# labhamlet/wavjepa

Hardware: AMD Instinct MI355X
Metric: jepa_pretrain_clips_per_sec (higher is better)
Workload: dtype bf16; 1 GPU; WavJEPA-base JEPA pre-training step, 2.01 s @16 kHz white-noise clips (32159 samples -> 200 tokens), 256 clips per GPU (32 sources x 8 crops), AudioSet masker, random-init weights; workload_name=2s-bf16, global_batch=256, seq_len=200, parallelism=dp1, persistent_gemm_workgroups_per_xcd=32

## Files before the change

include/wavjepa_hip.h:

```cpp
#ifndef WAVJEPA_HIP_H
#define WAVJEPA_HIP_H
#include <stdint.h>

#ifdef __cplusplus
extern "C" {
#endif

#define WJ_ABI_VERSION 17
int wj_abi_version(void);
int wj_device_count(void);
int wj_struct_size(const char* name);

enum {
    WJ_EPI_BF16 = 0,
    WJ_EPI_BIAS_GELU2 = 1,
    WJ_EPI_MUL_GELU_GRAD = 2,
    WJ_EPI_ADD_F32 = 3,
    WJ_EPI_ATOMIC_F32 = 4,
    WJ_EPI_CONV_GELU = 5,
    WJ_EPI_BIAS_GELU = 6,
    WJ_EPI_BF16_ADD_POS = 8,
    WJ_EPI_MUL_GELU_GRAD_Z = 7
};
typedef struct {
// ... 246 lines not shown
} wj_gelu_bwd_args;
int wj_gelu_bwd_bf16(const wj_gelu_bwd_args*, void* stream);

typedef struct {
    int64_t ticks;
} wj_spin_args;
int wj_spin(const wj_spin_args*, void* stream);


typedef struct {
    void* buf;
    const int32_t* rows;
    int32_t n_rows, row_bytes;
} wj_zero_rows_args;
int wj_zero_rows(const wj_zero_rows_args*, void* stream);

typedef struct {
    const void* src;
    void* dst;
    int32_t C_out, C_in, k, stride, rho, U, mode;
} wj_conv_w_args;
int wj_conv_weight_layout(const wj_conv_w_args*, void* stream);

typedef struct {
    const void* x;
    const float* pos;
    float* y_f32;
    void* y_bf16;
    int32_t M, T, D;
} wj_add_pos_args;
int wj_add_pos(const wj_add_pos_args*, void* stream);

typedef struct {
    const void* x;
    const int32_t* idx;
    void* out;
    int32_t n_rows, D, elem_bytes;
// ... 237 lines not shown
```

wavjepa_amd/csrc/conv0.hip:

```cpp
#include <string.h>
#include "common.h"
#include "../../include/wavjepa_hip.h"

namespace {

constexpr int TC = 256;
constexpr int NTH = 256;

struct Geo {
    int N, C_in, L, C, k, stride, L_out, P;
    long clip_stride;
};

template <int TAPS>
__device__ __forceinline__ void load_weights(float (&w)[4][TAPS], const bf16_t* __restrict__ wsrc, int c4) {
#pragma unroll
    for (int j = 0; j < 4; ++j)
#pragma unroll
        for (int tp = 0; tp < TAPS; ++tp) w[j][tp] = bf2f(wsrc[(long)(c4 + j) * TAPS + tp]);
}

__device__ __forceinline__ int stage_audio(float* xs, const bf16_t* __restrict__ audio, const Geo& g, int n, int t0, int span_max) {
    const int span = min(span_max, g.L - t0 * g.stride);
    for (int ci = 0; ci < g.C_in; ++ci)
// ... 44 lines not shown
    }
}

constexpr int STATS_SLOTS = 768;
inline int stats_tcs(int N, int L_out, int C_in) {
    static int forced = -1;
    if (forced < 0) forced = wj_lab_env_int("WJ_CONV0_STATS_TCS", 0);
    if (forced >= 32) return forced / 32 * 32;
    int chunks = (STATS_SLOTS + N / 2) / (N > 0 ? N : 1);
    const int most = (L_out + 255) / 256;
    chunks = chunks < 1 ? 1 : (chunks > most ? most : chunks);
    const int tcs = ((L_out + chunks - 1) / chunks + 31) / 32 * 32;
    const int cap = 2176 / (C_in > 0 ? C_in : 1) / 32 * 32;
    return tcs > cap ? (cap < 32 ? 32 : cap) : tcs;
}
template <int TAPS>
__global__ __launch_bounds__(256) void conv0_gram_kernel(const bf16_t* __restrict__ audio, double* __restrict__ part, Geo g, int span, int TCS) {
    extern __shared__ __attribute__((aligned(16))) bf16_t xa[];
    constexpr int G = TAPS + TAPS * TAPS;
    __shared__ double red[4][G];
    const int n = blockIdx.y, t0 = blockIdx.x * TCS;
    for (int ci = 0; ci < g.C_in; ++ci)
        for (int i = threadIdx.x; i < span; i += 256) {
            const long src = (long)t0 * g.stride + i;
            xa[ci * span + i] = src < g.L ? audio[(long)n * g.clip_stride + (long)ci * g.L + src] : f2bf(0.f);
        }
    __syncthreads();
    const int lane = threadIdx.x & 63, wave = threadIdx.x >> 6;
    const int tcount = min(TCS, g.L_out - t0);
    for (int p = lane; p < G; p += 64) {
        const bool one = p < TAPS;
        const int qa = one ? p : (p - TAPS) / TAPS, qb = one ? 0 : (p - TAPS) - qa * TAPS;
        const int ca = qa / g.k, cb = qb / g.k;
        const int offa = ca * span + (qa - ca * g.k), offb = cb * span + (qb - cb * g.k);
        double acc = 0.0;
        for (int t = wave; t < tcount; t += 4) {
            const float a = bf2f(xa[offa + t * g.stride]);
            const float b = one ? 1.0f : bf2f(xa[offb + t * g.stride]);
            acc += (double)(a * b);
        }
        red[wave][p] = acc;
    }
    __syncthreads();
    double* o = part + ((long)n * gridDim.x + blockIdx.x) * G;
    for (int p = threadIdx.x; p < G; p += 256) o[p] = (red[0][p] + red[1][p]) + (red[2][p] + red[3][p]);
}

__global__ __launch_bounds__(256) void conv0_fold_f64_kernel(const double* __restrict__ part, int chunks, int rec, double* __restrict__ out) {
    const int n = blockIdx.y;
    const double* src = part + (long)n * chunks * rec;
    for (int i = blockIdx.x * 256 + threadIdx.x; i < rec; i += gridDim.x * 256) {
        double s = 0.0;
        for (int ch = 0; ch < chunks; ++ch) s += src[(long)ch * rec + i];
        out[(long)n * rec + i] = s;
    }
}
// ... 568 lines not shown
```

wavjepa_amd/csrc/misc.hip:

```cpp
#include <string.h>
#include "common.h"
#include "../../include/wavjepa_hip.h"
#ifdef WJ_LAB
#include "../../include/wavjepa_hip_lab.h"
#endif

namespace {

inline int grid_for(long n_items, int per_block, int cap = 8192) {
    long g = (n_items + per_block - 1) / per_block;
    if (g < 1) g = 1;
    return (int)(g > cap ? cap : g);
}

__global__ __launch_bounds__(256) void gelu_bwd_kernel(const bf16_t* __restrict__ dpost, const bf16_t* __restrict__ pre,
                                                       bf16_t* __restrict__ dpre, long n8) {
    for (long i = blockIdx.x * 256L + threadIdx.x; i < n8; i += (long)gridDim.x * 256) {
        const bf16x8 d = *reinterpret_cast<const bf16x8*>(dpost + i * 8);
        const bf16x8 p = *reinterpret_cast<const bf16x8*>(pre + i * 8);
        bf16x8 o;
#pragma unroll
        for (int e = 0; e < 8; ++e) o[e] = f2bf(bf2f(d[e]) * gelu_grad_f(bf2f(p[e])));
        *reinterpret_cast<bf16x8*>(dpre + i * 8) = o;
    }
// ... 13 lines not shown
        for (int e = 0; e < 8; ++e) { o[e] = f2bf(bf2f(d[e]) * gelu_grad_f(bf2f(p[e]))); z[e] = f2bf(0.f); }
        *reinterpret_cast<bf16x8*>(dpre + off) = o;
        if (clear_dpost) *reinterpret_cast<bf16x8*>(dpost + off) = z;
    }
}

__global__ __launch_bounds__(256) void zero_rows_kernel(char* __restrict__ buf, const int32_t* __restrict__ rows, int n_rows,
                                                        int row16) {
    const long n = (long)n_rows * row16;
    for (long i = blockIdx.x * 256L + threadIdx.x; i < n; i += (long)gridDim.x * 256) {
        const int r = (int)(i / row16), c = (int)(i - (long)r * row16);
        *reinterpret_cast<uint4*>(buf + ((long)rows[r] * row16 + c) * 16) = make_uint4(0, 0, 0, 0);
    }
}

__global__ __launch_bounds__(256) void conv_w_kernel(wj_conv_w_args a) {
    const int Co = a.C_out, Ci = a.C_in, k = a.k;
    if (a.mode == 0) {
        const long n = (long)Co * Ci * k;
        for (long i = blockIdx.x * 256L + threadIdx.x; i < n; i += (long)gridDim.x * 256) {
            const int c = (int)(i % Ci);
            const int kk = (int)((i / Ci) % k);
            const int o = (int)(i / ((long)Ci * k));
            ((bf16_t*)a.dst)[i] = f2bf(((const float*)a.src)[((long)o * Ci + c) * k + kk]);
        }
    } else if (a.mode == 1) {
        const long n = (long)a.U * Co * Ci;
        for (long i = blockIdx.x * 256L + threadIdx.x; i < n; i += (long)gridDim.x * 256) {
            const int c = (int)(i % Ci);
            const int o = (int)((i / Ci) % Co);
            const int v = (int)(i / ((long)Ci * Co));
            const int kk = a.rho + a.stride * (a.U - 1 - v);
            ((bf16_t*)a.dst)[i] = f2bf(((const float*)a.src)[((long)o * Ci + c) * k + kk]);
        }
    } else {
        const long n = (long)Co * Ci * k;
        for (long i = blockIdx.x * 256L + threadIdx.x; i < n; i += (long)gridDim.x * 256) {
            const int kk = (int)(i % k);
            const int c = (int)((i / k) % Ci);
            const int o = (int)(i / ((long)Ci * k));
            ((float*)a.dst)[i] += ((const float*)a.src)[(long)o * Ci * k + (long)kk * Ci + c];
        }
    }
}

__global__ __launch_bounds__(256) void add_pos_kernel(wj_add_pos_args a) {
    const int D4 = a.D / 4;
    const long n = (long)a.M * D4;
    for (long i = blockIdx.x * 256L + threadIdx.x; i < n; i += (long)gridDim.x * 256) {
        const int m = (int)(i / D4), c = (int)(i - (long)m * D4) * 4;
        const bf16x4 x = *reinterpret_cast<const bf16x4*>((const bf16_t*)a.x + (long)m * a.D + c);
        const f32x4 p = *reinterpret_cast<const f32x4*>(a.pos + (long)(m % a.T) * a.D + c);
        f32x4 y;
        bf16x4 yb;
#pragma unroll
        for (int e = 0; e < 4; ++e) { y[e] = bf2f(x[e]) + p[e]; yb[e] = f2bf(y[e]); }
        if (a.y_f32) *reinterpret_cast<f32x4*>(a.y_f32 + (long)m * a.D + c) = y;
        if (a.y_bf16) *reinterpret_cast<bf16x4*>((bf16_t*)a.y_bf16 + (long)m * a.D + c) = yb;
// ... 452 lines not shown

extern "C" int wj_abi_version(void) { return WJ_ABI_VERSION; }
extern "C" int wj_device_count(void) {
    int n = 0;
    if (hipGetDeviceCount(&n) != hipSuccess) return 0;
    return n;
}

extern "C" int wj_struct_size(const char* name) {
    if (!name) return -1;
#define WJ_SZ(T) if (!strcmp(name, #T)) return (int)sizeof(T);
    WJ_SZ(wj_gemm_args) WJ_SZ(wj_ln_fwd_args) WJ_SZ(wj_ln_bwd_args) WJ_SZ(wj_ln_pre_fwd_args) WJ_SZ(wj_ln_pre_bwd_args) WJ_SZ(wj_colsum_args) WJ_SZ(wj_attn_fwd_args)
    WJ_SZ(wj_attn_bwd_args) WJ_SZ(wj_conv0_fwd_args) WJ_SZ(wj_conv0_bwd_args) WJ_SZ(wj_gelu_bwd_args) WJ_SZ(wj_conv_w_args)
    WJ_SZ(wj_add_pos_args) WJ_SZ(wj_gather_args) WJ_SZ(wj_scatter_fill_args) WJ_SZ(wj_scatter_fill_bwd_args)
    WJ_SZ(wj_unmask_rows_args) WJ_SZ(wj_instnorm_args) WJ_SZ(wj_mse_args) WJ_SZ(wj_ema_args) WJ_SZ(wj_sumsq_args)
    WJ_SZ(wj_adamw_args) WJ_SZ(wj_cast_args) WJ_SZ(wj_crop_args) WJ_SZ(wj_zero_rows_args) WJ_SZ(wj_instnorm_mean_args) WJ_SZ(wj_spin_args)
    WJ_SZ(wj_gemm_fp8_args) WJ_SZ(wj_quantize_fp8_args) WJ_SZ(wj_wgrad_group_args) WJ_SZ(wj_rir_conv_args) WJ_SZ(wj_snr_mix_args) WJ_SZ(wj_resample_args) WJ_SZ(wj_mse_groups_args) WJ_SZ(wj_transpose_args) WJ_SZ(wj_colsum_group_args) WJ_SZ(wj_rccl_init_args) WJ_SZ(wj_rccl_launch_args) WJ_SZ(wj_rccl_wait_args) WJ_SZ(wj_audio_prepare_args) WJ_SZ(wj_noise_prepare_args)
#ifdef WJ_LAB
    WJ_SZ(wj_collective_footprint_args)
#endif
#undef WJ_SZ
    return -1;
}

int64_t wj_gemm_ws_bytes(const wj_gemm_args* a);
int64_t wj_wgrad_group_ws_bytes(const wj_wgrad_group_args* a);
int64_t wj_colsum_bf16_ws_bytes(const wj_colsum_args* a);
int64_t wj_conv0_fwd_ws_bytes(const wj_conv0_fwd_args* a);
int64_t wj_conv0_bwd_ws_bytes(const wj_conv0_bwd_args* a);
int64_t wj_rir_conv_ws_bytes(const wj_rir_conv_args* a);
int64_t wj_snr_mix_ws_bytes(const wj_snr_mix_args* a);
// ... 19 lines not shown
    if (!strcmp(fn, "wj_conv0_gn_gelu_fwd")) return wj_conv0_fwd_ws_bytes((const wj_conv0_fwd_args*)args);
    if (!strcmp(fn, "wj_conv0_gn_gelu_bwd")) return wj_conv0_bwd_ws_bytes((const wj_conv0_bwd_args*)args);
    if (!strcmp(fn, "wj_masked_mse")) {
        const wj_mse_args* a = (const wj_mse_args*)args;
        return (2 + (int64_t)a->B * a->G * a->T) * 4;
    }
    if (!strcmp(fn, "wj_grad_sumsq")) return 1024 * 4;
    if (!strcmp(fn, "wj_rir_convolve")) return wj_rir_conv_ws_bytes((const wj_rir_conv_args*)args);
    if (!strcmp(fn, "wj_snr_mix")) return wj_snr_mix_ws_bytes((const wj_snr_mix_args*)args);
    if (!strcmp(fn, "wj_mse_groups")) return wj_mse_groups_ws_bytes((const wj_mse_groups_args*)args);
    if (!strcmp(fn, "wj_audio_prepare")) return wj_audio_prepare_ws_bytes((const wj_audio_prepare_args*)args);
    if (!strcmp(fn, "wj_noise_prepare")) return wj_noise_prepare_ws_bytes((const wj_noise_prepare_args*)args);
    static const char* const none[] = {"wj_layernorm_fwd", "wj_layernorm_pre_fwd", "wj_colsum_f32", "wj_attn_fwd", "wj_gelu_bwd_bf16",
        "wj_conv_weight_layout", "wj_add_pos", "wj_mask_gather_rows", "wj_mask_scatter_fill_pos",
        "wj_unmask_rows_f32", "wj_instnorm_accumulate", "wj_instnorm_mean", "wj_ema_update", "wj_adamw_step", "wj_cast_f32_to_bf16",
        "wj_crop_normalize_bf16", "wj_zero_rows", "wj_spin", "wj_gemm_mxfp8", "wj_quantize_mxfp8", "wj_resample_fir", "wj_transpose_bf16", "wj_colsum_f32_group", "wj_rccl_bucket_allreduce_launch", "wj_rccl_bucket_allreduce_wait", "wj_collective_footprint"};
    for (const char* n : none)
        if (!strcmp(fn, n)) return 0;
    return -1;
}

extern "C" int wj_gelu_bwd_bf16(const wj_gelu_bwd_args* a, void* stream) {
    WJ_CLEAR_STALE_ERROR();
    if (a && a->rows) {
        if (!a->dpost || !a->pre || !a->dpre || a->n_rows < 0 || a->row_elems <= 0 || (a->row_elems & 7)) return WJ_ERR_ARG;
        if (a->n_rows == 0) return WJ_OK;
        hipLaunchKernelGGL(gelu_bwd_rows_kernel, dim3(grid_for((long)a->n_rows * (a->row_elems / 8), 256)), dim3(256), 0, STREAM,
                           (bf16_t*)a->dpost, (const bf16_t*)a->pre, (bf16_t*)a->dpre, a->rows, a->n_rows, a->row_elems / 8,
                           a->clear_dpost);
        WJ_CHECK_LAUNCH();
        return WJ_OK;
// ... 60 lines not shown
    WJ_CHECK_LAUNCH();
    return WJ_OK;
}
#endif

extern "C" int wj_zero_rows(const wj_zero_rows_args* a, void* stream) {
    WJ_CLEAR_STALE_ERROR();
    if (!a || !a->buf || !a->rows || a->n_rows < 0 || a->row_bytes <= 0 || (a->row_bytes & 15)) return WJ_ERR_ARG;
    if (a->n_rows == 0) return WJ_OK;
    hipLaunchKernelGGL(zero_rows_kernel, dim3(grid_for((long)a->n_rows * (a->row_bytes / 16), 256)), dim3(256), 0, STREAM,
                       (char*)a->buf, a->rows, a->n_rows, a->row_bytes / 16);
    WJ_CHECK_LAUNCH();
    return WJ_OK;
}

extern "C" int wj_conv_weight_layout(const wj_conv_w_args* a, void* stream) {
    WJ_CLEAR_STALE_ERROR();
    if (!a || !a->src || !a->dst || a->C_out <= 0 || a->C_in <= 0 || a->k <= 0 || a->mode < 0 || a->mode > 2) return WJ_ERR_ARG;
    if (a->mode == 1 && (a->U <= 0 || a->rho < 0 || a->rho + a->stride * (a->U - 1) >= a->k)) return WJ_ERR_ARG;
    const long n = a->mode == 1 ? (long)a->U * a->C_out * a->C_in : (long)a->C_out * a->C_in * a->k;
    hipLaunchKernelGGL(conv_w_kernel, dim3(grid_for(n, 256, 2048)), dim3(256), 0, STREAM, *a);
    WJ_CHECK_LAUNCH();
    return WJ_OK;
}

extern "C" int wj_add_pos(const wj_add_pos_args* a, void* stream) {
    WJ_CLEAR_STALE_ERROR();
    if (!a || !a->x || !a->pos || a->M <= 0 || a->T <= 0 || a->D <= 0 || (a->D & 3)) return WJ_ERR_ARG;
    hipLaunchKernelGGL(add_pos_kernel, dim3(grid_for((long)a->M * a->D / 4, 256)), dim3(256), 0, STREAM, *a);
    WJ_CHECK_LAUNCH();
    return WJ_OK;
}

extern "C" int wj_mask_gather_rows(const wj_gather_args* a, void* stream) {
    WJ_CLEAR_STALE_ERROR();
    if (!a || !a->x || !a->idx || !a->out || a->n_rows < 0 || a->D <= 0) return WJ_ERR_ARG;
// ... 139 lines not shown
```

wavjepa_amd/engine.py:

```python
from __future__ import annotations

from dataclasses import dataclass
from typing import Dict, List, Optional, Sequence, Tuple

import numpy as np
import torch

from . import ops
from .params import FlatParams


def _empty(*shape, dtype, device):
    import os
    if os.environ.get("WJ_ARENA_FILL", "") == "nan":
        if not dtype.is_floating_point:
            return torch.full(shape, 0x7f, dtype=dtype, device=device)
        return torch.full(shape, float("nan"), dtype=dtype, device=device)
    return torch.empty(*shape, dtype=dtype, device=device)


@dataclass
class EngineConfig:
    conv_spec: Sequence[Tuple[int, int, int]]
    in_channels: int
# ... 250 lines not shown
        self.T = self.S * self.Tc
        self.stacks = list(cfg.conv_prefixes)
        assert len(self.stacks) in (1, self.S)
        self.C = cfg.conv_spec[-1][0]
        assert all(c == self.C for c, _, _ in cfg.conv_spec), "all conv layers must have the same width"
        assert cfg.d_enc % cfg.h_enc == 0 and cfg.d_dec % cfg.h_dec == 0
        self.N = 0
        self.G = 0
        import os as _os
        self.use_side = _os.environ.get("WJ_SIDE_STREAM", "1") != "0"
        self._opt_ev = None
        self.ragged = _os.environ.get("WJ_RAGGED", "1") != "0"
        self.ragged_step = False
        self.sparse_conv = _os.environ.get("WJ_SPARSE_CONV", "1") != "0" and all(k >= st for _, k, st in cfg.conv_spec[1:])
        self._conv_grads_dirty = False
        self.deterministic = _os.environ.get("WJ_DETERMINISTIC", "0") == "1"
        self._det_slab: Dict[str, torch.Tensor] = {}
        self.fuse_conv_gelu_bwd = _os.environ.get("WJ_FUSE_CONV_GELU_BWD", "1") != "0"
        self.trim_tail = _os.environ.get("WJ_TRIM_TAIL", "1") != "0"
        self.tail = None
        self.fp8 = _os.environ.get("WJ_FP8", "0") == "1"
        self._check_fp8()
        self._w8: Dict[int, Tuple[torch.Tensor, torch.Tensor, int, int]] = {}
        self._a8: Dict[str, Tuple[torch.Tensor, torch.Tensor]] = {}
        self.side = self._pick_side_stream() if self.use_side else torch.cuda.Stream(device=self.dev)
        self.has_mapper = "post_extraction_mapper.weight" in flat.by_name
        self.wt_dgrad = _os.environ.get("WJ_WT_DGRAD", "1") != "0"
        self.pair_split = _os.environ.get("WJ_PAIR_SPLIT", "0") == "1"
        self.pair_ws = None
        self._conv_w_fresh = False
# ... 149 lines not shown
                mine.copy_(src.reshape(mine.shape))
        if force_cast or not f.bf16_fresh:
            ops.cast_f32_to_bf16(f.p32, f.p16, f.n)
            if f.tn > 0:
                ops.cast_f32_to_bf16(f.t32, f.t16, f.tn)
            f.bf16_fresh = True
        if self.fp8:
            self._fp8_weights()
        self._wt_fresh = None
        self._conv_w_fresh = False

    def _conv_weight_layouts(self) -> None:
        if self._conv_w_fresh:
            return
        f, C = self.flat, self.C
        for si, pre in enumerate(self.stacks):
            for l, (_, k, s) in enumerate(self.cfg.conv_spec):
                if l == 0:
                    continue
                src = f.ptr32(f"{pre}{l}.0.weight")
                ops.conv_weight_layout(src, self._conv_w[f"{si}:wp{l}"], C_out=C, C_in=C, k=k, mode=0)
                for rho in range(s):
                    U = len(range(rho, k, s))
                    if U > 0:
                        ops.conv_weight_layout(src, self._conv_w[f"{si}:wd{l}_{rho}"], C_out=C, C_in=C, k=k, mode=1, stride=s, rho=rho, U=U)
        self._conv_w_fresh = True

    def _rows(self, nrows: int, width: int, dtype, lead: int = 2, tail: int = 8) -> Tuple[torch.Tensor, int]:
        t = torch.zeros((lead + nrows + tail) * width, dtype=dtype, device=self.dev)
        return t, t.data_ptr() + lead * width * t.element_size()

    def _alloc_stack(self, M: int, D: int, H: int, B: int, layers: int) -> List[_Acts]:
        bf, f32, dev = torch.bfloat16, torch.float32, self.dev
        out = []
        for _ in range(layers):
            a = _Acts()
            a.qkv = _empty(M, 3 * D, dtype=bf, device=dev)
            a.o = _empty(M, D, dtype=bf, device=dev)
            a.lse = _empty(B * H * self.T, dtype=f32, device=dev)
            a.p = _empty(M, D, dtype=bf, device=dev)
# ... 28 lines not shown
            if need >= full:
                return full
            return min(full, max((int(need * margin) + 255) // 256 * 256, old if same else 0))

        self.cap_enc = cap(need_enc, full_enc, getattr(self, "cap_enc", 0))
        self.cap_dec = cap(need_dec, full_dec, getattr(self, "cap_dec", 0))
        c, bf, f32, dev = self.cfg, torch.bfloat16, torch.float32, self.dev
        T, C = self.T, self.C
        M, Mp = N * T, N * G * T
        self.N, self.G, self.M, self.Mp = N, G, M, Mp
        self._train_alloc = train
        Me, Md = self.cap_enc, self.cap_dec
        nl = len(c.conv_spec)
        Nc = N * self.S
        self.post, self.post_ptr, self.pre, self.pre_ptr = [], [], [None], [0]
        self.dpost, self.dpost_ptr, self.dpre, self.dpre_ptr = [], [], [None], [0]
        for l in range(nl):
            t, p = self._rows(Nc * self.P[l], C, bf)
            self.post.append(t); self.post_ptr.append(p)
            if l > 0:
                t, p = self._rows(Nc * self.P[l], C, bf)
                self.pre.append(t); self.pre_ptr.append(p)
            if train:
                t, p = self._rows(Nc * self.P[l], C, bf)
                self.dpost.append(t); self.dpost_ptr.append(p)
                if l > 0:
                    t, p = self._rows(Nc * self.P[l], C, bf)
                    self.dpre.append(t); self.dpre_ptr.append(p)
        if self.pair_split and self.pair_ws is None:
            self.pair_ws = torch.zeros(ops.workspace_bytes("wj_gemm_bf16", M=256 * (self.PAIR_TILES[1] // 2), N=512, K=2048, lda=2048, ldb=2048,
# ... 287 lines not shown
        if not self.use_side:
            fn()
            return
        main = torch.cuda.current_stream()
        ev = torch.cuda.Event()
        ev.record(main)
        self.side.wait_event(ev)
        with torch.cuda.stream(self.side):
            fn()

    def optimizer_on_side(self, fn) -> None:
        self._opt_main = torch.cuda.current_stream()
        self._on_side(fn)
        self._opt_ev = torch.cuda.Event()
        self._opt_ev.record(self.side)

    def wait_optimizer(self) -> None:
        if self._opt_ev is not None:
            cur = torch.cuda.current_stream()
            cur.wait_event(self._opt_ev)
            if getattr(self, "_opt_main", None) is None or cur == self._opt_main:
                self._opt_ev = None

    def _join_side(self) -> None:
        if self.use_side:
            ev = torch.cuda.Event()
            ev.record(self.side)
            torch.cuda.current_stream().wait_event(ev)

    def _layer_bwd(self, w: _Layer, a: _Acts, x_in: torch.Tensor, xb_in: torch.Tensor, dy: torch.Tensor, dyb: Optional[torch.Tensor],
# ... 473 lines not shown
            if not self.has_mapper:
                ops.unmask_rows_f32(dy, plan.inv, self.d_fn, M=M, D=De, src_is_f32=True)
                dy = self.d_fn
        else:
            ops.cast_f32_to_bf16(dy, self.d_lf_b, M * De)
        if self.has_mapper:
            self._colsum_bf16(self.d_lf_b, f.gptr("post_extraction_mapper.bias"), M=M, N=De, ldx=De)
            self._wgrad(self.d_lf_b, self.fn_b, f.gptr("post_extraction_mapper.weight"), De, C, M)
            ops.gemm(self.d_lf_b, f.ptr16("post_extraction_mapper.weight"), self.d_fn, M=M, N=C, K=De, lda=De, ldb=C, ldc=C,
                     b_trans=1, epilogue=ops.EPI_ADD_F32)
            d_fn = self.d_fn
        else:
            d_fn = dy
        nl = len(c.conv_spec)
        S, Tc = self.S, self.Tc
        self._ln_bwd_direct(d_fn, self.post_ptr[-1], f.ptr32("feature_norms.weight"), self.fn_mean, self.fn_rstd, M=M, D=C,
                            ds_bf16=self.dpost_ptr[-1], dgamma=f.gptr("feature_norms.weight"), dbeta=f.gptr("feature_norms.bias"),
                            x_is_bf16=True, in_seg=self.P[-1], in_valid=Tc, out_seg=self.P[-1], out_valid=Tc, chan=S if S > 1 else 0)
        sparse = rag and self.sparse_conv
        if sparse:
            act_rows = self._conv_rows(plan)
            if self._conv_grads_dirty:
                for t in self.dpost + self.dpre[1:]:
                    t.zero_()
                self._conv_grads_dirty = False
        else:
            self._conv_grads_dirty = True
        groups = self._stack_groups()
        side_wgrad = sparse and self.use_side and self.conv_wgrad_side
        late_clear = []
        for l in range(nl - 1, 0, -1):
            _, k, s = c.conv_spec[l]
            empty_phase = any(len(range(rho, k, s)) == 0 for rho in range(s))
            if empty_phase:
                self.dpost[l - 1].zero_()
            for gi, (si, c0, nclips) in enumerate(groups):
                rows = nclips * self.P[l]
                r0, r0p = c0 * self.P[l] * C * 2, c0 * self.P[l - 1] * C * 2
                dwp = self._conv_w[f"{si}:dwp{l}"]
                if not side_wgrad:
                    dwp.zero_()
                if sparse:
                    act, n_act, ext, n_ext = act_rows[l][gi]
                    if not (self.fuse_conv_gelu_bwd and l < nl - 1):
                        ops.gelu_bwd_bf16(self.dpost_ptr[l], self.pre_ptr[l], self.dpre_ptr[l], 0, rows=act, n_rows=n_act, row_elems=C,
# ... 17 lines not shown
                for rho in range(s):
                    U = len(range(rho, k, s))
                    if U == 0:
                        continue
                    if sparse:
                        if n_ext > 0 and self.fuse_conv_gelu_bwd and l - 1 >= 1:
                            ops.gemm(self.dpre_ptr[l] - (U - 1) * C * 2, self._conv_w[f"{si}:wd{l}_{rho}"], self.dpre_ptr[l - 1] + rho * C * 2,
                                     M=n_ext, N=C, K=U * C, lda=C, ldb=C, ldc=s * C, b_trans=1, rowmap=ext,
                                     epilogue=ops.EPI_MUL_GELU_GRAD_Z, aux=self.pre_ptr[l - 1] + rho * C * 2)
                        elif n_ext > 0:
                            ops.gemm(self.dpre_ptr[l] - (U - 1) * C * 2, self._conv_w[f"{si}:wd{l}_{rho}"], self.dpost_ptr[l - 1] + rho * C * 2,
                                     M=n_ext, N=C, K=U * C, lda=C, ldb=C, ldc=s * C, b_trans=1, rowmap=ext)
                    else:
                        ops.gemm(self.dpre_ptr[l] + r0 - (U - 1) * C * 2, self._conv_w[f"{si}:wd{l}_{rho}"],
                                 self.dpost_ptr[l - 1] + r0p + rho * C * 2, M=rows, N=C, K=U * C, lda=C, ldb=C, ldc=s * C, b_trans=1)
                if sparse and side_wgrad:
                    late_clear.append((self.dpre_ptr[l], act, n_act))
                elif sparse:
                    ops.zero_rows(self.dpre_ptr[l], act, n_rows=n_act, row_bytes=C * 2)
        _, k0, s0 = c.conv_spec[0]
        audio_p = self.audio.data_ptr()
        for ch in range(S):
            pre = self.stacks[min(ch, len(self.stacks) - 1)]
            c0 = ch * N
            lists = {}
            if sparse:
                rows0, n0, off0, max0 = act_rows[0][ch]
                lists = dict(rows=rows0, row_off=off0, max_rows=max0)
            ops.conv0_bwd(audio_p + ch * c.n_samples * 2 if S > 1 else self.audio, f.ptr16(f"{pre}0.0.weight"), f.ptr32(f"{pre}0.2.weight"),
                          f.ptr32(f"{pre}0.2.bias"), self.gn_stats[0, c0:], self.gn_stats[1, c0:], self.dpost_ptr[0] + c0 * self.P[0] * C * 2,
                          f.gptr(f"{pre}0.0.weight"), f.gptr(f"{pre}0.2.weight"), f.gptr(f"{pre}0.2.bias"), self.gn_ws_b,
                          yx=self.gn_yx[c0:], x1=self.gn_x1[c0:], N=N, C_in=c.in_channels, L=c.n_samples, C=C, k=k0, stride=s0,
                          L_out=self.L[0], P=self.P[0], audio_clip_stride=S * c.in_channels * c.n_samples if S > 1 else 0, **lists)
            if sparse:
                ops.zero_rows(self.dpost_ptr[0] + c0 * self.P[0] * C * 2, rows0, n_rows=n0, row_bytes=C * 2)
        if late_clear:
            self._join_side()
            for ptr, act, n_act in late_clear:
                ops.zero_rows(ptr, act, n_rows=n_act, row_bytes=C * 2)

    def _conv_rows(self, plan: MaskPlan):
        cached = getattr(plan, "_conv_rows", None)
        if cached is not None and cached[0] == (self.N, self.S, len(self.stacks), tuple(self.P)):
            return cached[1]
        N, S = self.N, self.S
        keep = (plan.ctx_u8.cpu().numpy() == 0) if plan.ctx_np is None else ~plan.ctx_np
        if S > 1:
            keep = np.ascontiguousarray(keep.reshape(N, S, self.Tc).transpose(1, 0, 2)).reshape(S * N, self.Tc)
        lists = conv_active_rows(keep, self.P, self.cfg.conv_spec)
        pad = np.zeros(256, np.int32)
        act0, off0 = lists[0]
        host, keys = [], []
        for l, (act, ext) in lists.items():
            if l == 0:
# ... 63 lines not shown
```

wavjepa_amd/ops.py:

```python
from __future__ import annotations

import ctypes
from typing import Optional, Union

import torch

from . import _abi
from ._abi import ENUMS, STRUCTS

Ptr = Union[torch.Tensor, int, None]

EPI_BF16 = ENUMS["WJ_EPI_BF16"]
EPI_BIAS_GELU2 = ENUMS["WJ_EPI_BIAS_GELU2"]
EPI_MUL_GELU_GRAD = ENUMS["WJ_EPI_MUL_GELU_GRAD"]
EPI_ADD_F32 = ENUMS["WJ_EPI_ADD_F32"]
EPI_ATOMIC_F32 = ENUMS["WJ_EPI_ATOMIC_F32"]
EPI_CONV_GELU = ENUMS["WJ_EPI_CONV_GELU"]
EPI_BIAS_GELU = ENUMS["WJ_EPI_BIAS_GELU"]
EPI_MUL_GELU_GRAD_Z = ENUMS["WJ_EPI_MUL_GELU_GRAD_Z"]
EPI_BF16_ADD_POS = ENUMS["WJ_EPI_BF16_ADD_POS"]
GROUP_STATS_SPLIT = _abi.DEFINES["WJ_GROUP_STATS_SPLIT"]
COLSUM_GROUP_MAX = _abi.DEFINES["WJ_COLSUM_GROUP_MAX"]


def _p(x: Ptr) -> int:
    if x is None:
        return 0
    if isinstance(x, int):
        return x
    return x.data_ptr()


def _stream() -> int:
    return torch.cuda.current_stream().cuda_stream


PROFILE = None
# ... 312 lines not shown

def spin(ticks: int, stream: Optional[int] = None) -> None:
    _run("wj_spin", "wj_spin_args", stream, ticks=int(ticks))


def collective_footprint(buf: Ptr, nbytes: int, *, workgroups: int = 32, passes: int = 2, min_ticks: int = 0,
                         stream: Optional[int] = None) -> None:
    _run("wj_collective_footprint", "wj_collective_footprint_args", stream, _lab=True, buf=_p(buf), bytes=int(nbytes), min_ticks=int(min_ticks),
         workgroups=int(workgroups), passes=int(passes))


def zero_rows(buf: Ptr, rows: Ptr, *, n_rows: int, row_bytes: int, stream: Optional[int] = None) -> None:
    _run("wj_zero_rows", "wj_zero_rows_args", stream, buf=_p(buf), rows=_p(rows), n_rows=n_rows, row_bytes=row_bytes)


def conv_weight_layout(src: Ptr, dst: Ptr, *, C_out: int, C_in: int, k: int, mode: int, stride: int = 1, rho: int = 0,
                       U: int = 1, stream: Optional[int] = None) -> None:
    _run("wj_conv_weight_layout", "wj_conv_w_args", stream, src=_p(src), dst=_p(dst), C_out=C_out, C_in=C_in, k=k,
         stride=stride, rho=rho, U=U, mode=mode)


def add_pos(x: Ptr, pos: Ptr, *, M: int, T: int, D: int, y_f32: Ptr = None, y_bf16: Ptr = None,
            stream: Optional[int] = None) -> None:
    _run("wj_add_pos", "wj_add_pos_args", stream, x=_p(x), pos=_p(pos), y_f32=_p(y_f32), y_bf16=_p(y_bf16), M=M, T=T, D=D)


def mask_gather_rows(x: Ptr, idx: Ptr, out: Ptr, *, n_rows: int, D: int, elem_bytes: int, stream: Optional[int] = None) -> None:
    _run("wj_mask_gather_rows", "wj_gather_args", stream, x=_p(x), idx=_p(idx), out=_p(out), n_rows=n_rows, D=D,
         elem_bytes=elem_bytes)

# ... 116 lines not shown
```

Measured before the change: 5590 clips/s.

## Batch conv weight layouts and row clears, defer clears to side stream, rework gram kernel

Conv weight relayout calls are batched into grouped kernel launches, and the sparse row-zeroing calls are collected into grouped launches. Those clears can be deferred to the side stream after the optimizer update and waited on at the next backward. The conv0 gram kernel is rewritten so each thread accumulates the symmetric upper-triangle products in registers, with wave-shuffle reductions replacing one-product-per-lane loops. The goal is fewer launches and less serial work on the main stream, at the cost of extra cross-stream event handling and higher register pressure in the gram kernel.

```diff
diff --git a/include/wavjepa_hip.h b/include/wavjepa_hip.h
--- a/include/wavjepa_hip.h
+++ b/include/wavjepa_hip.h
@@ -284,6 +284,15 @@
     int32_t n_rows, row_bytes;
 } wj_zero_rows_args;
 int wj_zero_rows(const wj_zero_rows_args*, void* stream);
+#define WJ_ZERO_ROWS_GROUP_MAX 8
+typedef struct {
+    void* buf[WJ_ZERO_ROWS_GROUP_MAX];
+    const int32_t* rows[WJ_ZERO_ROWS_GROUP_MAX];
+    int32_t n_rows[WJ_ZERO_ROWS_GROUP_MAX], row_bytes[WJ_ZERO_ROWS_GROUP_MAX];
+    int32_t n;
+    int32_t workgroups;
+} wj_zero_rows_group_args;
+int wj_zero_rows_group(const wj_zero_rows_group_args*, void* stream);
 
 typedef struct {
     const void* src;
@@ -291,6 +300,15 @@
     int32_t C_out, C_in, k, stride, rho, U, mode;
 } wj_conv_w_args;
 int wj_conv_weight_layout(const wj_conv_w_args*, void* stream);
+#define WJ_CONV_W_GROUP_MAX 64
+typedef struct {
+    const void* src[WJ_CONV_W_GROUP_MAX];
+    void* dst[WJ_CONV_W_GROUP_MAX];
+    int32_t C_out[WJ_CONV_W_GROUP_MAX], C_in[WJ_CONV_W_GROUP_MAX], k[WJ_CONV_W_GROUP_MAX], stride[WJ_CONV_W_GROUP_MAX];
+    int32_t rho[WJ_CONV_W_GROUP_MAX], U[WJ_CONV_W_GROUP_MAX], mode[WJ_CONV_W_GROUP_MAX];
+    int32_t n;
+} wj_conv_w_group_args;
+int wj_conv_weight_layout_group(const wj_conv_w_group_args*, void* stream);
 
 typedef struct {
     const void* x;
diff --git a/wavjepa_amd/csrc/conv0.hip b/wavjepa_amd/csrc/conv0.hip
--- a/wavjepa_amd/csrc/conv0.hip
+++ b/wavjepa_amd/csrc/conv0.hip
@@ -82,6 +82,54 @@
     const int cap = 2176 / (C_in > 0 ? C_in : 1) / 32 * 32;
     return tcs > cap ? (cap < 32 ? 32 : cap) : tcs;
 }
+template <int TAPS, int R0, int R1, bool X1>
+__device__ __forceinline__ void gram_rows(const bf16_t* xa, const int (&off)[TAPS], int stride, int tcount, double* red) {
+    constexpr int NE = (R1 - R0) * TAPS - (R1 * (R1 - 1) - R0 * (R0 - 1)) / 2;
+    double acc[NE], x1[X1 ? TAPS : 1];
+#pragma unroll
+    for (int e = 0; e < NE; ++e) acc[e] = 0.0;
+#pragma unroll
+    for (int q = 0; q < (X1 ? TAPS : 1); ++q) x1[q] = 0.0;
+    for (int t = threadIdx.x; t < tcount; t += 256) {
+        double x[TAPS];
+#pragma unroll
+        for (int q = X1 ? 0 : R0; q < TAPS; ++q) x[q] = (double)bf2f(xa[off[q] + t * stride]);
+        int e = 0;
+#pragma unroll
+        for (int qa = R0; qa < R1; ++qa)
+#pragma unroll
+            for (int qb = qa; qb < TAPS; ++qb) { acc[e] = fma(x[qa], x[qb], acc[e]); ++e; }
+        if (X1) {
+#pragma unroll
+            for (int q = 0; q < TAPS; ++q) x1[q] += x[q];
+        }
+    }
+#pragma unroll
+    for (int m = 32; m >= 1; m >>= 1) {
+#pragma unroll
+        for (int e = 0; e < NE; ++e) acc[e] += __shfl_xor(acc[e], m, 64);
+        if (X1) {
+#pragma unroll
+            for (int q = 0; q < TAPS; ++q) x1[q] += __shfl_xor(x1[q], m, 64);
+        }
+    }
+    if ((threadIdx.x & 63) == 0) {
+        int e = 0;
+#pragma unroll
+        for (int qa = R0; qa < R1; ++qa)
+#pragma unroll
+            for (int qb = qa; qb < TAPS; ++qb) {
+                red[TAPS + qa * TAPS + qb] = acc[e];
+                red[TAPS + qb * TAPS + qa] = acc[e];
+                ++e;
+            }
+        if (X1) {
+#pragma unroll
+            for (int q = 0; q < TAPS; ++q) red[q] = x1[q];
+        }
+    }
+}
+
 template <int TAPS>
 __global__ __launch_bounds__(256) void conv0_gram_kernel(const bf16_t* __restrict__ audio, double* __restrict__ part, Geo g, int span, int TCS) {
     extern __shared__ __attribute__((aligned(16))) bf16_t xa[];
@@ -94,20 +142,24 @@
             xa[ci * span + i] = src < g.L ? audio[(long)n * g.clip_stride + (long)ci * g.L + src] : f2bf(0.f);
         }
     __syncthreads();
-    const int lane = threadIdx.x & 63, wave = threadIdx.x >> 6;
+    const int wave = threadIdx.x >> 6;
     const int tcount = min(TCS, g.L_out - t0);
-    for (int p = lane; p < G; p += 64) {
-        const bool one = p < TAPS;
-        const int qa = one ? p : (p - TAPS) / TAPS, qb = one ? 0 : (p - TAPS) - qa * TAPS;
-        const int ca = qa / g.k, cb = qb / g.k;
-        const int offa = ca * span + (qa - ca * g.k), offb = cb * span + (qb - cb * g.k);
-        double acc = 0.0;
-        for (int t = wave; t < tcount; t += 4) {
-            const float a = bf2f(xa[offa + t * g.stride]);
-            const float b = one ? 1.0f : bf2f(xa[offb + t * g.stride]);
-            acc += (double)(a * b);
-        }
-        red[wave][p] = acc;
+    int off[TAPS];
+#pragma unroll
+    for (int q = 0; q < TAPS; ++q) {
+        const int ci = q / g.k;
+        off[q] = ci * span + (q - ci * g.k);
+    }
+    if constexpr (TAPS == 10) {
+        gram_rows<TAPS, 0, 4, false>(xa, off, g.stride, tcount, red[wave]);
+        gram_rows<TAPS, 4, 10, true>(xa, off, g.stride, tcount, red[wave]);
+    } else {
+        static_assert(TAPS == 20, "row passes are laid out for 20 taps");
+        gram_rows<TAPS, 0, 4, false>(xa, off, g.stride, tcount, red[wave]);
+        gram_rows<TAPS, 4, 8, false>(xa, off, g.stride, tcount, red[wave]);
+        gram_rows<TAPS, 8, 12, false>(xa, off, g.stride, tcount, red[wave]);
+        gram_rows<TAPS, 12, 16, false>(xa, off, g.stride, tcount, red[wave]);
+        gram_rows<TAPS, 16, 20, true>(xa, off, g.stride, tcount, red[wave]);
     }
     __syncthreads();
     double* o = part + ((long)n * gridDim.x + blockIdx.x) * G;
diff --git a/wavjepa_amd/csrc/misc.hip b/wavjepa_amd/csrc/misc.hip
--- a/wavjepa_amd/csrc/misc.hip
+++ b/wavjepa_amd/csrc/misc.hip
@@ -51,11 +51,30 @@
     }
 }
 
-__global__ __launch_bounds__(256) void conv_w_kernel(wj_conv_w_args a) {
+struct ZeroRowsGroup {
+    char* buf[WJ_ZERO_ROWS_GROUP_MAX];
+    const int32_t* rows[WJ_ZERO_ROWS_GROUP_MAX];
+    long start[WJ_ZERO_ROWS_GROUP_MAX + 1];
+    int row16[WJ_ZERO_ROWS_GROUP_MAX];
+    int n;
+};
+__global__ __launch_bounds__(256) void zero_rows_group_kernel(ZeroRowsGroup a) {
+    const long total = a.start[a.n];
+    for (long i = blockIdx.x * 256L + threadIdx.x; i < total; i += (long)gridDim.x * 256) {
+        int it = 0;
+        while (it + 1 < a.n && i >= a.start[it + 1]) ++it;
+        const long j = i - a.start[it];
+        const int row16 = a.row16[it];
+        const int r = (int)(j / row16), c = (int)(j - (long)r * row16);
+        *reinterpret_cast<uint4*>(a.buf[it] + ((long)a.rows[it][r] * row16 + c) * 16) = make_uint4(0, 0, 0, 0);
+    }
+}
+
+__device__ __forceinline__ void conv_w_body(const wj_conv_w_args& a, int blk, int nblk) {
     const int Co = a.C_out, Ci = a.C_in, k = a.k;
     if (a.mode == 0) {
         const long n = (long)Co * Ci * k;
-        for (long i = blockIdx.x * 256L + threadIdx.x; i < n; i += (long)gridDim.x * 256) {
+        for (long i = blk * 256L + threadIdx.x; i < n; i += (long)nblk * 256) {
             const int c = (int)(i % Ci);
             const int kk = (int)((i / Ci) % k);
             const int o = (int)(i / ((long)Ci * k));
@@ -63,7 +82,7 @@
         }
     } else if (a.mode == 1) {
         const long n = (long)a.U * Co * Ci;
-        for (long i = blockIdx.x * 256L + threadIdx.x; i < n; i += (long)gridDim.x * 256) {
+        for (long i = blk * 256L + threadIdx.x; i < n; i += (long)nblk * 256) {
             const int c = (int)(i % Ci);
             const int o = (int)((i / Ci) % Co);
             const int v = (int)(i / ((long)Ci * Co));
@@ -72,13 +91,26 @@
         }
     } else {
         const long n = (long)Co * Ci * k;
-        for (long i = blockIdx.x * 256L + threadIdx.x; i < n; i += (long)gridDim.x * 256) {
+        for (long i = blk * 256L + threadIdx.x; i < n; i += (long)nblk * 256) {
             const int kk = (int)(i % k);
             const int c = (int)((i / k) % Ci);
             const int o = (int)(i / ((long)Ci * k));
             ((float*)a.dst)[i] += ((const float*)a.src)[(long)o * Ci * k + (long)kk * Ci + c];
         }
     }
+}
+
+__global__ __launch_bounds__(256) void conv_w_kernel(wj_conv_w_args a) { conv_w_body(a, blockIdx.x, gridDim.x); }
+
+struct ConvWGroup {
+    wj_conv_w_args p[WJ_CONV_W_GROUP_MAX];
+    int start[WJ_CONV_W_GROUP_MAX + 1];
+    int n;
+};
+__global__ __launch_bounds__(256) void conv_w_group_kernel(ConvWGroup a) {
+    int p = 0;
+    while (p + 1 < a.n && (int)blockIdx.x >= a.start[p + 1]) ++p;
+    conv_w_body(a.p[p], blockIdx.x - a.start[p], a.start[p + 1] - a.start[p]);
 }
 
 __global__ __launch_bounds__(256) void add_pos_kernel(wj_add_pos_args a) {
@@ -561,7 +593,7 @@
     WJ_SZ(wj_attn_bwd_args) WJ_SZ(wj_conv0_fwd_args) WJ_SZ(wj_conv0_bwd_args) WJ_SZ(wj_gelu_bwd_args) WJ_SZ(wj_conv_w_args)
     WJ_SZ(wj_add_pos_args) WJ_SZ(wj_gather_args) WJ_SZ(wj_scatter_fill_args) WJ_SZ(wj_scatter_fill_bwd_args)
     WJ_SZ(wj_unmask_rows_args) WJ_SZ(wj_instnorm_args) WJ_SZ(wj_mse_args) WJ_SZ(wj_ema_args) WJ_SZ(wj_sumsq_args)
-    WJ_SZ(wj_adamw_args) WJ_SZ(wj_cast_args) WJ_SZ(wj_crop_args) WJ_SZ(wj_zero_rows_args) WJ_SZ(wj_instnorm_mean_args) WJ_SZ(wj_spin_args)
+    WJ_SZ(wj_adamw_args) WJ_SZ(wj_cast_args) WJ_SZ(wj_crop_args) WJ_SZ(wj_zero_rows_args) WJ_SZ(wj_zero_rows_group_args) WJ_SZ(wj_conv_w_group_args) WJ_SZ(wj_instnorm_mean_args) WJ_SZ(wj_spin_args)
     WJ_SZ(wj_gemm_fp8_args) WJ_SZ(wj_quantize_fp8_args) WJ_SZ(wj_wgrad_group_args) WJ_SZ(wj_rir_conv_args) WJ_SZ(wj_snr_mix_args) WJ_SZ(wj_resample_args) WJ_SZ(wj_mse_groups_args) WJ_SZ(wj_transpose_args) WJ_SZ(wj_colsum_group_args) WJ_SZ(wj_rccl_init_args) WJ_SZ(wj_rccl_launch_args) WJ_SZ(wj_rccl_wait_args) WJ_SZ(wj_audio_prepare_args) WJ_SZ(wj_noise_prepare_args)
 #ifdef WJ_LAB
     WJ_SZ(wj_collective_footprint_args)
@@ -611,7 +643,7 @@
     static const char* const none[] = {"wj_layernorm_fwd", "wj_layernorm_pre_fwd", "wj_colsum_f32", "wj_attn_fwd", "wj_gelu_bwd_bf16",
         "wj_conv_weight_layout", "wj_add_pos", "wj_mask_gather_rows", "wj_mask_scatter_fill_pos",
         "wj_unmask_rows_f32", "wj_instnorm_accumulate", "wj_instnorm_mean", "wj_ema_update", "wj_adamw_step", "wj_cast_f32_to_bf16",
-        "wj_crop_normalize_bf16", "wj_zero_rows", "wj_spin", "wj_gemm_mxfp8", "wj_quantize_mxfp8", "wj_resample_fir", "wj_transpose_bf16", "wj_colsum_f32_group", "wj_rccl_bucket_allreduce_launch", "wj_rccl_bucket_allreduce_wait", "wj_collective_footprint"};
+        "wj_crop_normalize_bf16", "wj_zero_rows", "wj_zero_rows_group", "wj_conv_weight_layout_group", "wj_spin", "wj_gemm_mxfp8", "wj_quantize_mxfp8", "wj_resample_fir", "wj_transpose_bf16", "wj_colsum_f32_group", "wj_rccl_bucket_allreduce_launch", "wj_rccl_bucket_allreduce_wait", "wj_collective_footprint"};
     for (const char* n : none)
         if (!strcmp(fn, n)) return 0;
     return -1;
@@ -702,12 +734,60 @@
     return WJ_OK;
 }
 
+extern "C" int wj_zero_rows_group(const wj_zero_rows_group_args* a, void* stream) {
+    WJ_CLEAR_STALE_ERROR();
+    if (!a || a->n < 1 || a->n > WJ_ZERO_ROWS_GROUP_MAX || a->workgroups < 0) return WJ_ERR_ARG;
+    ZeroRowsGroup g;
+    memset(&g, 0, sizeof(g));
+    for (int i = 0; i < a->n; ++i) {
+        if (a->n_rows[i] < 0 || a->row_bytes[i] <= 0 || (a->row_bytes[i] & 15)) return WJ_ERR_ARG;
+        if (a->n_rows[i] == 0) continue;
+        if (!a->buf[i] || !a->rows[i]) return WJ_ERR_ARG;
+        g.buf[g.n] = (char*)a->buf[i];
+        g.rows[g.n] = a->rows[i];
+        g.row16[g.n] = a->row_bytes[i] / 16;
+        g.start[g.n + 1] = g.start[g.n] + (long)a->n_rows[i] * (a->row_bytes[i] / 16);
+        ++g.n;
+    }
+    if (g.n == 0) return WJ_OK;
+    const int grid = a->workgroups > 0 ? grid_for(g.start[g.n], 256, a->workgroups) : grid_for(g.start[g.n], 256);
+    hipLaunchKernelGGL(zero_rows_group_kernel, dim3(grid), dim3(256), 0, STREAM, g);
+    WJ_CHECK_LAUNCH();
+    return WJ_OK;
+}
+
+static bool conv_w_args_ok(const wj_conv_w_args* a) {
+    if (!a->src || !a->dst || a->C_out <= 0 || a->C_in <= 0 || a->k <= 0 || a->mode < 0 || a->mode > 2) return false;
+    if (a->mode == 1 && (a->U <= 0 || a->rho < 0 || a->rho + a->stride * (a->U - 1) >= a->k)) return false;
+    return true;
+}
+static int conv_w_blocks(const wj_conv_w_args* a) {
+    const long n = a->mode == 1 ? (long)a->U * a->C_out * a->C_in : (long)a->C_out * a->C_in * a->k;
+    return grid_for(n, 256, 2048);
+}
+
 extern "C" int wj_conv_weight_layout(const wj_conv_w_args* a, void* stream) {
     WJ_CLEAR_STALE_ERROR();
-    if (!a || !a->src || !a->dst || a->C_out <= 0 || a->C_in <= 0 || a->k <= 0 || a->mode < 0 || a->mode > 2) return WJ_ERR_ARG;
-    if (a->mode == 1 && (a->U <= 0 || a->rho < 0 || a->rho + a->stride * (a->U - 1) >= a->k)) return WJ_ERR_ARG;
-    const long n = a->mode == 1 ? (long)a->U * a->C_out * a->C_in : (long)a->C_out * a->C_in * a->k;
-    hipLaunchKernelGGL(conv_w_kernel, dim3(grid_for(n, 256, 2048)), dim3(256), 0, STREAM, *a);
+    if (!a || !conv_w_args_ok(a)) return WJ_ERR_ARG;
+    hipLaunchKernelGGL(conv_w_kernel, dim3(conv_w_blocks(a)), dim3(256), 0, STREAM, *a);
+    WJ_CHECK_LAUNCH();
+    return WJ_OK;
+}
+
+extern "C" int wj_conv_weight_layout_group(const wj_conv_w_group_args* a, void* stream) {
+    WJ_CLEAR_STALE_ERROR();
+    if (!a || a->n < 1 || a->n > WJ_CONV_W_GROUP_MAX) return WJ_ERR_ARG;
+    ConvWGroup g;
+    memset(&g, 0, sizeof(g));
+    g.n = a->n;
+    for (int i = 0; i < a->n; ++i) {
+        wj_conv_w_args& p = g.p[i];
+        p.src = a->src[i]; p.dst = a->dst[i];
+        p.C_out = a->C_out[i]; p.C_in = a->C_in[i]; p.k = a->k[i]; p.stride = a->stride[i]; p.rho = a->rho[i]; p.U = a->U[i]; p.mode = a->mode[i];
+        if (!conv_w_args_ok(&p)) return WJ_ERR_ARG;
+        g.start[i + 1] = g.start[i] + conv_w_blocks(&p);
+    }
+    hipLaunchKernelGGL(conv_w_group_kernel, dim3(g.start[g.n]), dim3(256), 0, STREAM, g);
     WJ_CHECK_LAUNCH();
     return WJ_OK;
 }
diff --git a/wavjepa_amd/engine.py b/wavjepa_amd/engine.py
--- a/wavjepa_amd/engine.py
+++ b/wavjepa_amd/engine.py
@@ -288,6 +288,10 @@
         self.ragged_step = False
         self.sparse_conv = _os.environ.get("WJ_SPARSE_CONV", "1") != "0" and all(k >= st for _, k, st in cfg.conv_spec[1:])
         self._conv_grads_dirty = False
+        self.defer_row_clears = True
+        self.row_clear_wgs = 256
+        self._row_clears = None
+        self._side_update_seen = False
         self.deterministic = _os.environ.get("WJ_DETERMINISTIC", "0") == "1"
         self._det_slab: Dict[str, torch.Tensor] = {}
         self.fuse_conv_gelu_bwd = _os.environ.get("WJ_FUSE_CONV_GELU_BWD", "1") != "0"
@@ -467,16 +471,19 @@
         if self._conv_w_fresh:
             return
         f, C = self.flat, self.C
+        items = []
         for si, pre in enumerate(self.stacks):
             for l, (_, k, s) in enumerate(self.cfg.conv_spec):
                 if l == 0:
                     continue
                 src = f.ptr32(f"{pre}{l}.0.weight")
-                ops.conv_weight_layout(src, self._conv_w[f"{si}:wp{l}"], C_out=C, C_in=C, k=k, mode=0)
+                items.append(dict(src=src, dst=self._conv_w[f"{si}:wp{l}"], C_out=C, C_in=C, k=k, mode=0))
                 for rho in range(s):
                     U = len(range(rho, k, s))
                     if U > 0:
-                        ops.conv_weight_layout(src, self._conv_w[f"{si}:wd{l}_{rho}"], C_out=C, C_in=C, k=k, mode=1, stride=s, rho=rho, U=U)
+                        items.append(dict(src=src, dst=self._conv_w[f"{si}:wd{l}_{rho}"], C_out=C, C_in=C, k=k, mode=1, stride=s, rho=rho, U=U))
+        for i in range(0, len(items), ops.CONV_W_GROUP_MAX):
+            ops.conv_weight_layout_group(items[i:i + ops.CONV_W_GROUP_MAX])
         self._conv_w_fresh = True
 
     def _rows(self, nrows: int, width: int, dtype, lead: int = 2, tail: int = 8) -> Tuple[torch.Tensor, int]:
@@ -535,6 +542,8 @@
         nl = len(c.conv_spec)
         Nc = N * self.S
         self.post, self.post_ptr, self.pre, self.pre_ptr = [], [], [None], [0]
+        if self._row_clears is not None and self._row_clears["ev"] is None:
+            self._row_clears = None
         self.dpost, self.dpost_ptr, self.dpre, self.dpre_ptr = [], [], [None], [0]
         for l in range(nl):
             t, p = self._rows(Nc * self.P[l], C, bf)
@@ -852,6 +861,28 @@
         self._on_side(fn)
         self._opt_ev = torch.cuda.Event()
         self._opt_ev.record(self.side)
+        self._side_update_seen = True
+        if self._row_clears is not None and self._row_clears["ev"] is None:
+            with torch.cuda.stream(self.side):
+                self._issue_row_clears(self._row_clears["items"], self.row_clear_wgs)
+                self._row_clears["ev"] = torch.cuda.Event()
+                self._row_clears["ev"].record(self.side)
+
+    @staticmethod
+    def _issue_row_clears(items, workgroups: int = 0) -> None:
+        for i in range(0, len(items), ops.ZERO_ROWS_GROUP_MAX):
+            ops.zero_rows_group(items[i:i + ops.ZERO_ROWS_GROUP_MAX], workgroups=workgroups)
+
+    def _settle_row_clears(self) -> None:
+        rc = self._row_clears
+        if rc is None:
+            return
+        if rc["ev"] is None:
+            self._issue_row_clears(rc["items"])
+            self._side_update_seen = False
+        else:
+            torch.cuda.current_stream().wait_event(rc["ev"])
+        self._row_clears = None
 
     def wait_optimizer(self) -> None:
         if self._opt_ev is not None:
@@ -1355,6 +1386,7 @@
             d_fn = dy
         nl = len(c.conv_spec)
         S, Tc = self.S, self.Tc
+        self._settle_row_clears()
         self._ln_bwd_direct(d_fn, self.post_ptr[-1], f.ptr32("feature_norms.weight"), self.fn_mean, self.fn_rstd, M=M, D=C,
                             ds_bf16=self.dpost_ptr[-1], dgamma=f.gptr("feature_norms.weight"), dbeta=f.gptr("feature_norms.bias"),
                             x_is_bf16=True, in_seg=self.P[-1], in_valid=Tc, out_seg=self.P[-1], out_valid=Tc, chan=S if S > 1 else 0)
@@ -1369,7 +1401,7 @@
             self._conv_grads_dirty = True
         groups = self._stack_groups()
         side_wgrad = sparse and self.use_side and self.conv_wgrad_side
-        late_clear = []
+        clears = []
         for l in range(nl - 1, 0, -1):
             _, k, s = c.conv_spec[l]
             empty_phase = any(len(range(rho, k, s)) == 0 for rho in range(s))
@@ -1417,10 +1449,8 @@
                     else:
                         ops.gemm(self.dpre_ptr[l] + r0 - (U - 1) * C * 2, self._conv_w[f"{si}:wd{l}_{rho}"],
                                  self.dpost_ptr[l - 1] + r0p + rho * C * 2, M=rows, N=C, K=U * C, lda=C, ldb=C, ldc=s * C, b_trans=1)
-                if sparse and side_wgrad:
-                    late_clear.append((self.dpre_ptr[l], act, n_act))
-                elif sparse:
-                    ops.zero_rows(self.dpre_ptr[l], act, n_rows=n_act, row_bytes=C * 2)
+                if sparse:
+                    clears.append((self.dpre_ptr[l], act, n_act, C * 2))
         _, k0, s0 = c.conv_spec[0]
         audio_p = self.audio.data_ptr()
         for ch in range(S):
@@ -1436,11 +1466,15 @@
                           yx=self.gn_yx[c0:], x1=self.gn_x1[c0:], N=N, C_in=c.in_channels, L=c.n_samples, C=C, k=k0, stride=s0,
                           L_out=self.L[0], P=self.P[0], audio_clip_stride=S * c.in_channels * c.n_samples if S > 1 else 0, **lists)
             if sparse:
-                ops.zero_rows(self.dpost_ptr[0] + c0 * self.P[0] * C * 2, rows0, n_rows=n0, row_bytes=C * 2)
-        if late_clear:
+                clears.append((self.dpost_ptr[0] + c0 * self.P[0] * C * 2, rows0, n0, C * 2))
+        if not clears:
+            return
+        if self.defer_row_clears and self.use_side and self._side_update_seen:
+            self._row_clears = dict(items=clears, keep=(act_rows, self.dpost, self.dpre), ev=None)
+            return
+        if side_wgrad:
             self._join_side()
-            for ptr, act, n_act in late_clear:
-                ops.zero_rows(ptr, act, n_rows=n_act, row_bytes=C * 2)
+        self._issue_row_clears(clears)
 
     def _conv_rows(self, plan: MaskPlan):
         cached = getattr(plan, "_conv_rows", None)
diff --git a/wavjepa_amd/ops.py b/wavjepa_amd/ops.py
--- a/wavjepa_amd/ops.py
+++ b/wavjepa_amd/ops.py
@@ -21,6 +21,8 @@
 EPI_BF16_ADD_POS = ENUMS["WJ_EPI_BF16_ADD_POS"]
 GROUP_STATS_SPLIT = _abi.DEFINES["WJ_GROUP_STATS_SPLIT"]
 COLSUM_GROUP_MAX = _abi.DEFINES["WJ_COLSUM_GROUP_MAX"]
+CONV_W_GROUP_MAX = _abi.DEFINES["WJ_CONV_W_GROUP_MAX"]
+ZERO_ROWS_GROUP_MAX = _abi.DEFINES["WJ_ZERO_ROWS_GROUP_MAX"]
 
 
 def _p(x: Ptr) -> int:
@@ -363,6 +365,36 @@
     _run("wj_zero_rows", "wj_zero_rows_args", stream, buf=_p(buf), rows=_p(rows), n_rows=n_rows, row_bytes=row_bytes)
 
 
+def _run_group(fn: str, a, fields: dict, stream: Optional[int]) -> None:
+    s = _stream() if stream is None else stream
+    if PROFILE is None:
+        _abi.call(fn, a, s)
+        return
+    e0, e1 = TimingEvent(), TimingEvent()
+    e0.record(s)
+    _abi.call(fn, a, s)
+    e1.record(s)
+    PROFILE.append((fn, fields, e0, e1))
+
+
+def zero_rows_group(items, *, workgroups: int = 0, stream: Optional[int] = None) -> None:
+    a = STRUCTS["wj_zero_rows_group_args"]()
+    for i, (buf, rows, n_rows, row_bytes) in enumerate(items[:len(a.buf)]):
+        a.buf[i], a.rows[i], a.n_rows[i], a.row_bytes[i] = _p(buf), _p(rows), n_rows, row_bytes
+    a.n, a.workgroups = len(items), int(workgroups)
+    _run_group("wj_zero_rows_group", a, dict(n=len(items), workgroups=int(workgroups)), stream)
+
+
+def conv_weight_layout_group(items, stream: Optional[int] = None) -> None:
+    a = STRUCTS["wj_conv_w_group_args"]()
+    for i, it in enumerate(items[:len(a.src)]):
+        a.src[i], a.dst[i] = _p(it["src"]), _p(it["dst"])
+        a.C_out[i], a.C_in[i], a.k[i], a.mode[i] = it["C_out"], it["C_in"], it["k"], it["mode"]
+        a.stride[i], a.rho[i], a.U[i] = it.get("stride", 1), it.get("rho", 0), it.get("U", 0)
+    a.n = len(items)
+    _run_group("wj_conv_weight_layout_group", a, dict(n=len(items)), stream)
+
+
 def conv_weight_layout(src: Ptr, dst: Ptr, *, C_out: int, C_in: int, k: int, mode: int, stride: int = 1, rho: int = 0,
                        U: int = 1, stream: Optional[int] = None) -> None:
     _run("wj_conv_weight_layout", "wj_conv_w_args", stream, src=_p(src), dst=_p(dst), C_out=C_out, C_in=C_in, k=k,
```

Result: no change. 5608 clips/s, median of 6 (+0.3%).
